# JohnLonginotto/uq

Hardware: AMD Instinct MI355X
Metric: FASTQ encode MB/s (150bp synthetic; bit-exact tables vs reference) (higher is better)
Workload: dtype u8

## Files before the change

include/uqhip.h:

```cpp
#ifndef UQHIP_H
#define UQHIP_H
#include <stddef.h>
#include <stdint.h>

#ifdef __cplusplus
extern "C" {
#endif

#define UQ_ABI_VERSION 1
#define UQ_NONE UINT64_MAX

typedef struct uq_ctx uq_ctx;

const char* uq_last_error(void);
int uq_abi_version(void);
int uq_device_count(int* h_count);
int uq_ctx_create(int device, void* stream, uq_ctx** out);
int uq_ctx_destroy(uq_ctx* ctx);
int uq_ctx_reserve(uq_ctx* ctx, size_t scratch_bytes);
int uq_ctx_sync(uq_ctx* ctx);
int uq_dev_alloc(uq_ctx* ctx, size_t bytes, void** d_out);
int uq_dev_free(uq_ctx* ctx, void* d_ptr);
int uq_h2d(uq_ctx* ctx, void* d_dst, const void* h_src, size_t bytes);
int uq_d2h(uq_ctx* ctx, void* h_dst, const void* d_src, size_t bytes);
// ... 149 lines not shown
int uq_owner_of_rows(uq_ctx* ctx, const int64_t* d_row_index, uint64_t n, const int64_t* h_shard_starts, uint32_t world, uint8_t* d_owner);
int uq_index_affine(uq_ctx* ctx, const void* d_in, int in_itemsize, uint64_t n, int64_t add, void* d_out, int out_itemsize);
int uq_invert_permutation(uq_ctx* ctx, const void* d_perm, int perm_itemsize, uint64_t n, int64_t base, uint32_t* d_inv, uint64_t* h_bad);
int uq_scatter_rows(uq_ctx* ctx, const uint8_t* d_values, uint64_t n, uint32_t cols, const void* d_index, int index_itemsize, int64_t base,
                    uint64_t out_rows, uint8_t* d_out, uint64_t* h_bad);

#define UQ_QF_MAXC 8
#define UQ_QF_MAXT 24
typedef struct uq_qname_fused {
    uint32_t ok, plen, slen, nsep, l1len;
    uint32_t flags;
    uint32_t sample_step, nth;
    uint8_t line1[256];
    uint8_t seps[32];
    uint8_t inset[256];
    uint32_t vmin[UQ_QF_MAXC], vmax[UQ_QF_MAXC];
    uint32_t undetermined[UQ_QF_MAXC];
    uint64_t nreads;
    uint64_t thresholds[UQ_QF_MAXT];
    uint64_t counts[UQ_QF_MAXC][UQ_QF_MAXT];
} uq_qname_fused;
int uq_qname_guess(uq_ctx* ctx, const uint8_t* d_buf, const uint64_t* d_line_start, uint64_t nreads, uq_qname_fused* d_q);
int uq_qname_guess_async(uq_ctx* ctx, const uint8_t* d_buf, const uint64_t* d_line_start, uq_qname_fused* d_q);
int uq_pack_stats_qname(uq_ctx* ctx, const uint8_t* d_buf, const uint64_t* d_line_start, uint64_t first_read, uint64_t nreads,
                        const uq_pack_params* h_guess, uint8_t* d_dna, uint8_t* d_qual, uint64_t* d_bad, uq_stats* d_stats,
                        uq_qname_fused* d_q, uint32_t* d_vals, uint64_t vals_pitch, int* h_fused);
int uq_pack_stats_qname_async(uq_ctx* ctx, const uint8_t* d_buf, const uint64_t* d_line_start, uint64_t capacity_reads,
                              const uq_pack_params* h_guess, uint8_t* d_dna, uint8_t* d_qual, uint64_t* d_bad, uq_stats* d_stats,
                              uq_qname_fused* d_q, uint32_t* d_vals, uint64_t vals_pitch, int* h_fused);
int uq_qname_fused_finish(uq_ctx* ctx, uq_qname_fused* d_q, const uint32_t* d_vals, uint64_t vals_pitch);
int uq_qname_fused_fetch(uq_ctx* ctx, const uq_qname_fused* d_q, uq_qname_fused* h_out);
int uq_qname_fused_first_seen(uq_ctx* ctx, const uint32_t* d_vals, uint64_t vals_pitch, uint64_t nreads, uint64_t read_offset,
                              const uint32_t* h_vmin, const uint32_t* h_range, int ncols, int64_t* d_first);
int uq_encode_u32(uq_ctx* ctx, const uint32_t* d_val, uint64_t n, uint32_t sub, int itemsize, void* d_out);
int uq_encode_u32_columns(uq_ctx* ctx, const uint32_t* d_vals, uint64_t vals_pitch, uint64_t n, int ncols, const uint32_t* h_sub,
                          const int* h_itemsize, void* const* h_d_outs);

typedef struct uq_decisions {
    uint32_t status, nbases, nquals, nall, nnq, ncand;
    uint8_t bases[256], qualities[256], all_bases[256];
    uint8_t nq_base[256]; int32_t nq_code[256];
    int32_t total_quals, bits_per_base, bits_per_quality, variable, dna_max, dna_min, dna_bytes_per_row, quality_bytes_per_row;
    uint64_t base_tot[256], qual_tot[256];
} uq_decisions;
int uq_decide_from_stats(const uq_stats_compact* h_compact, const uint64_t* h_dense, uint32_t len_min, uint32_t len_max, int notricks, int pad,
                         const uint64_t* h_first_seen, uq_decisions* h_out);
// ... 112 lines not shown
```

uq_amd/_lib.py:

```python
import ctypes as C
import os

HERE = os.path.dirname(os.path.abspath(__file__))
LIB_PATH = os.environ.get('UQ_LIB_PATH') or os.path.join(HERE, 'libuqhip.so')
UQ_NONE = (1 << 64) - 1
ABI_VERSION = 1


class UqHipError(RuntimeError):
    pass


class Stats(C.Structure):
    _fields_ = [('counts', C.c_uint64 * 65536), ('bad_plus', C.c_uint64), ('bad_len', C.c_uint64),
                ('len_min', C.c_uint32), ('len_max', C.c_uint32), ('max_record_bytes', C.c_uint32),
                ('reserved', C.c_uint32)]


class PackParams(C.Structure):
    _fields_ = [('dna_code', C.c_int16 * 256), ('qual_code', C.c_int16 * 256), ('n_qual', C.c_int32 * 256),
                ('bits_per_base', C.c_int32), ('bits_per_quality', C.c_int32), ('variable', C.c_int32),
                ('dna_bytes_per_row', C.c_int32), ('quality_bytes_per_row', C.c_int32),
                ('max_record_bytes', C.c_int32), ('dna_max', C.c_int32), ('avg_record_bytes', C.c_int32)]

# ... 124 lines not shown
    'uq_narrow': [_vp, _vp, _u64, _int, _vp],
    'uq_stack_columns': [_vp, _P(_vp), _P(_int), _int, _u64, _int, _vp],
    'uq_unstack_column': [_vp, _vp, _u64, _int, _int, _int, _int, _vp],
    'uq_unpack': [_vp, _vp, _vp, _u64, _P(UnpackParams), _vp, _vp, _vp, _vp],
    'uq_qname_analyse': [_vp, _vp, _u64, _P(_vp), _P(_int)],
    'uq_qname_json': [_vp, _P(C.c_char_p)],
    'uq_qname_column': [_vp, _int, _vp, _u64],
    'uq_qname_free': [_vp],
    'uq_qname_layout': [_vp, _vp, _vp, _u64, _u64, _vp, _u32, _P(QnameLayoutResult)],
    'uq_qname_tokenise': [_vp, _vp, _vp, _u64, _u32, _u32, _vp, _u32, _P(_vp), _P(_vp), _P(QnameColsResult)],
    'uq_prefix_distinct': [_vp, _vp, _int, _vp, _u64, _P(_u64), _int, _P(_u64)],
    'uq_int_prefix_distinct': [_vp, _vp, _u64, C.c_int64, _u64, _u64, _P(_u64), _int, _P(_u64)],
    'uq_encode_int': [_vp, _vp, _u64, C.c_int64, _int, _vp],
    'uq_unique_sorted_rows': [_vp, _vp, _u64, _u32, _vp, _vp, _P(_u64)],
    'uq_unique_rows_of_groups': [_vp, _vp, _u64, _u32, _vp, _vp, _u64, _vp],
    'uq_partition_order': [_vp, _vp, _u64, _u32, _vp, _vp, _P(_u64)],
    'uq_partition_rows': [_vp, _vp, _u32, _u32, _vp, _u64, _u64, _u64, _vp],
    'uq_owner_of_rows': [_vp, _vp, _u64, _P(C.c_int64), _u32, _vp],
    'uq_index_affine': [_vp, _vp, _int, _u64, C.c_int64, _vp, _int],
    'uq_invert_permutation': [_vp, _vp, _int, _u64, C.c_int64, _vp, _P(_u64)],
    'uq_scatter_rows': [_vp, _vp, _u64, _u32, _vp, _int, C.c_int64, _u64, _vp, _P(_u64)],
    'uq_qname_guess': [_vp, _vp, _vp, _u64, _vp],
    'uq_qname_guess_async': [_vp, _vp, _vp, _vp],
    'uq_pack_stats_qname': [_vp, _vp, _vp, _u64, _u64, _P(PackParams), _vp, _vp, _vp, _vp, _vp, _vp, _u64, _P(_int)],
    'uq_pack_stats_qname_async': [_vp, _vp, _vp, _u64, _P(PackParams), _vp, _vp, _vp, _vp, _vp, _vp, _u64, _P(_int)],
    'uq_qname_fused_finish': [_vp, _vp, _vp, _u64],
    'uq_qname_fused_fetch': [_vp, _vp, _P(QnameFused)],
    'uq_qname_fused_first_seen': [_vp, _vp, _u64, _u64, _u64, _P(_u32), _P(_u32), _int, _vp],
    'uq_encode_u32': [_vp, _vp, _u64, _u32, _int, _vp],
    'uq_encode_u32_columns': [_vp, _vp, _u64, _u64, _int, _P(_u32), _P(_int), _P(_vp)],
    'uq_decide_from_stats': [_vp, _vp, _u32, _u32, _int, _int, _vp, _P(Decisions)],
    'uq_make_pack_params': [C.c_char_p, _u32, C.c_char_p, _u32, C.c_char_p, _P(C.c_int32), _u32] + [C.c_int32] * 8 + [_P(PackParams)],
    'uq_same_pack_params': [_P(PackParams), _P(PackParams), _P(_int)],
    'uq_qname_fused_columns': [_P(QnameFused), _u64, _P(QnameColumns)],
    'uq_emit_fastq': [_vp, _P(EmitParams), _P(_vp), _P(_vp), _P(_vp), _vp, _vp, _vp, _u64, _vp, _vp, _u64, _P(_u64)],
    'uq_debug_scribble_lds': [_vp, C.c_uint32],
    'uq_sort_config': [_vp, C.c_int64, _P(_int), _int],
    'uq_sort_counters': [_vp, _P(_u64), _P(_u64)],
    'uq_decode_fastq': [_vp, _P(EmitParams), _P(UnpackParams), _P(_vp), _P(_vp), _P(_vp), _vp, _vp, _u64, _vp, _vp, _vp, _vp, _u64, _P(_u64), _P(_u64)],
    'uq_synth_size': [_vp, _P(SynthSpec), _u64, _u64, _P(_u64)],
    'uq_synth_fastq': [_vp, _P(SynthSpec), _u64, _u64, _vp, _u64],
    'uq_gzip_scan': [_vp, _u64, _vp, _u64, _P(_u64), _P(_u64), _P(_int), _P(_u64)],
    'uq_inflate_members': [_vp, _vp, _u64, _vp, _u64, _vp, _u64, _vp],
    'uq_inflate_member_host': [_vp, _u64, _vp, _u64, _u32, _P(_u32)],
    'uq_gzip_stream_begin': [_vp, _vp, _u64, _u64, _vp, _u64, _P(_vp), _P(_u64), _P(_u32), _P(_u64)],
    'uq_gzip_stream_finish': [_vp, _vp, _u64, _P(_u32), _P(_u64)],
# ... 54 lines not shown
```

uq_amd/csrc/api.hip:

```cpp
#include <stdarg.h>
#include "common.h"

static thread_local char g_err[1024] = "";

void uq_set_error(const char* fmt, ...) {
    va_list ap;
    va_start(ap, fmt);
    vsnprintf(g_err, sizeof(g_err), fmt, ap);
    va_end(ap);
}

extern "C" const char* uq_last_error(void) { return g_err; }
extern "C" int uq_abi_version(void) { return UQ_ABI_VERSION; }

extern "C" int uq_device_count(int* h_count) {
    UQ_REQUIRE(h_count, "uq_device_count: null out pointer");
    UQ_CHECK_HIP(hipGetDeviceCount(h_count));
    return 0;
}

extern "C" int uq_ctx_create(int device, void* stream, uq_ctx** out) {
    UQ_REQUIRE(out, "uq_ctx_create: null out pointer");
    int n = 0;
    UQ_CHECK_HIP(hipGetDeviceCount(&n));
// ... 5 lines not shown
    if (stream) { c->stream = (hipStream_t)stream; c->own_stream = false; }
    else { UQ_CHECK_HIP(hipStreamCreateWithFlags(&c->stream, hipStreamNonBlocking)); c->own_stream = true; }
    UQ_CHECK_HIP(hipEventCreate(&c->ev0));
    UQ_CHECK_HIP(hipEventCreate(&c->ev1));
    UQ_CHECK_HIP(hipHostMalloc((void**)&c->h_pinned, 131072, hipHostMallocDefault));
    UQ_CHECK_HIP(hipHostGetDevicePointer((void**)&c->d_pinned, c->h_pinned, 0));
    UQ_CHECK_HIP(hipMalloc((void**)&c->d_async, 64));
    *out = c;
    return 0;
}

extern "C" int uq_ctx_destroy(uq_ctx* c) {
    if (!c) return 0;
    (void)hipSetDevice(c->device);
    (void)hipStreamSynchronize(c->stream);
    if (c->scratch) (void)hipFree(c->scratch);
    if (c->idx_partials) (void)hipFree(c->idx_partials);
    if (c->idx_bitmap) (void)hipFree(c->idx_bitmap);
    if (c->scan_ws) (void)hipFree(c->scan_ws);
    if (c->h_pinned) (void)hipHostFree(c->h_pinned);
    if (c->d_async) (void)hipFree(c->d_async);
    if (c->qf_first) (void)hipFree(c->qf_first);
    if (c->qf_lay) (void)hipFree(c->qf_lay);
    if (c->d_compact) (void)hipFree(c->d_compact);
    (void)hipEventDestroy(c->ev0);
    (void)hipEventDestroy(c->ev1);
    if (c->own_stream) (void)hipStreamDestroy(c->stream);
    delete c;
    return 0;
}

namespace {
__global__ void read_back_kernel(const uint32_t* __restrict__ src, uint32_t* __restrict__ dst, uint32_t nwords) {
    for (uint32_t i = blockIdx.x * blockDim.x + threadIdx.x; i < nwords; i += gridDim.x * blockDim.x) dst[i] = src[i];
}
}

int uq_read_back(uq_ctx* c, void* h_dst, const void* d_src, size_t bytes) {
    const size_t off = (size_t)((const uint8_t*)h_dst - (const uint8_t*)c->h_pinned);
    UQ_REQUIRE(bytes % 4 == 0 && off % 4 == 0 && off + bytes <= 131072, "uq_read_back: destination outside the pinned staging buffer");
    if (bytes == 0) return 0;
    const uint32_t nwords = (uint32_t)(bytes / 4);
    read_back_kernel<<<nwords > 1024 ? 8 : 1, 256, 0, c->stream>>>((const uint32_t*)d_src, (uint32_t*)((uint8_t*)c->d_pinned + off), nwords);
    UQ_LAUNCH_CHECK();
    return 0;
}
// ... 93 lines not shown
```

uq_amd/csrc/common.h:

```cpp
#pragma once
#include <hip/hip_runtime.h>
#include <stdint.h>
#include <stdio.h>
#include <string.h>
#include "../../include/uqhip.h"

#define UQ_WAVE 64
#define UQ_NUM_CU 256

struct uq_ctx {
    int device;
    hipStream_t stream;
    bool own_stream;
    void* scratch;
    size_t scratch_bytes;
    hipEvent_t ev0, ev1;
    const uint8_t* idx_buf; uint64_t idx_nbytes; uint64_t idx_nlines;
    uint32_t* idx_partials; size_t idx_partials_cap;
    uint16_t* idx_bitmap;
    uint64_t* h_pinned;
    uint64_t* d_pinned;
    void* scan_ws; size_t scan_ws_bytes;
    unsigned long long* d_async;
    const uint8_t* async_buf; uint64_t async_nbytes; bool async_read;
    bool census_begun; uint64_t census_nb;
    uint32_t* qf_first;
    void* qf_lay; bool qf_lay_dirty;
    bool qf_dirty;
    const void* pk_stats; const void* pk_q; const void* stats_sent;
    uq_stats_compact* d_compact;
    const void* qf_sent;
    long long msd_min_rows; int msd_levels; int msd_bits[4];
    unsigned long long n_msd_rounds, n_lsd_rounds;
    const void* kreg_key[8]; int kreg_val[8]; int kreg_n;
    bool qf_attr_set;
};

void uq_set_error(const char* fmt, ...);

#define UQ_CHECK_HIP(expr)                                                              \
    do {                                                                                \
        hipError_t _e = (expr);                                                         \
        if (_e != hipSuccess) {                                                         \
            uq_set_error("%s failed: %s (%s:%d)", #expr, hipGetErrorString(_e), __FILE__, __LINE__); \
            return 1;                                                                   \
        }                                                                               \
    } while (0)

#define UQ_REQUIRE(cond, ...)                                                           \
    do {                                                                                \
// ... 88 lines not shown
```

uq_amd/csrc/qname_fused.hip:

```cpp
#include "common.h"
#include "lines.h"
#include "stats_compact.h"

namespace {
constexpr int QF_THREADS = 256;
constexpr int QF_MAXCH = 64;
constexpr uint32_t QF_SAMPLES = 4096;
constexpr uint32_t QF_ROW = 64, QF_STRIDE = QF_ROW + 4;
constexpr uint32_t QF_FT = 1u << 20;
constexpr uint32_t QF_SMALL = 4096;
constexpr size_t QF_PINNED_AT = 5200;
static_assert(sizeof(uq_qname_fused) % 4 == 0 && QF_PINNED_AT * 8 + sizeof(uq_qname_fused) <= 8000 * 8, "the structure's slot in the pinned staging");
constexpr uint64_t QF_PREFIX = 1ull << 21;

struct DevLine1 {
    uint8_t text[256];
    uint8_t slot[256];
    uint8_t ch[QF_MAXCH];
    uint16_t cnt[QF_MAXCH];
    uint16_t lastpos[QF_MAXCH];
    uint32_t len, nch, bad, pad;
};

__device__ __forceinline__ void stage_line(uint8_t* row, const uint8_t* q, uint32_t ql, const uint8_t* buf_end) {
    for (uint32_t c = 0; c < ql; c += 16) {
        if (q + c + 16 <= buf_end) {
            uint4 v;
            __builtin_memcpy(&v, q + c, 16);
            uint32_t* d = (uint32_t*)(row + c);
            d[0] = v.x; d[1] = v.y; d[2] = v.z; d[3] = v.w;
        } else {
            for (uint32_t b = c; b < ql; ++b) row[b] = q[b];
        }
    }
}

constexpr uint32_t QF_SPW = 8;
__global__ __launch_bounds__(64) void qname_sample_kernel(const uint8_t* __restrict__ buf, const uint64_t* __restrict__ ls, uint64_t n,
                                                                   const unsigned long long* __restrict__ d_async, uq_qname_layout_result* __restrict__ lay,
                                                                   DevLine1* __restrict__ l1_out, uint32_t* __restrict__ step_out, CensusView cv, uint64_t nbytes,
                                                                   const uint32_t* __restrict__ over) {
    __shared__ __align__(16) uint8_t stage[64 * QF_STRIDE];
    __shared__ DevLine1 l1;
    __shared__ unsigned long long s_entry[QF_MAXCH], s_viol[QF_MAXCH];
    __shared__ uint32_t s_lcp, s_lcs, s_flags;
    const uint32_t tid = threadIdx.x;
    const bool lists = cv.list != nullptr;
    uint64_t nlines = 4 * n;
    if (d_async) { nlines = d_async[0]; n = (d_async[1] || (lists && *over)) ? 0 : d_async[0] / 4; }
    uint32_t len = 0;
    if (n) { bool ok; const uint64_t e = lists ? cv_line_start(cv, nlines, 0, 0, 1, ok) : ls[1]; len = e >= 1 && e <= 256 ? (uint32_t)(e - 1) : 0xFFFFFFFFu; }
    for (uint32_t x = tid; x < 256; x += 64) { l1.text[x] = (len != 0xFFFFFFFFu && x < len) ? buf[x] : 0; l1.slot[x] = 0xFF; }
    if (tid < QF_MAXCH) { l1.ch[tid] = 0; l1.cnt[tid] = 0; l1.lastpos[tid] = 0; s_entry[tid] = UQ_NONE; s_viol[tid] = 0; }
    if (tid == 0) { s_lcp = 0xFFFFFFFFu; s_lcs = 0xFFFFFFFFu; s_flags = 0; }
    __syncthreads();
    const bool bad0 = len == 0 || len == 0xFFFFFFFFu || l1.text[0] != '@';
    if (!bad0 && len <= 64) {
        const uint32_t lane0 = lane_id();
        const uint32_t mych = lane0 < len ? (uint32_t)l1.text[lane0] : 0x100u;
        unsigned long long same = 0;
        for (uint32_t j = 0; j < len; ++j) {
            const unsigned long long bm = __ballot(mych == (uint32_t)__builtin_amdgcn_readlane((int)mych, (int)j));
            if (lane0 == j) same = bm;
        }
        const bool first = lane0 < len && (uint32_t)__builtin_ctzll(same | (1ull << 63)) == lane0;
        const unsigned long long fm = __ballot(first);
        if (first) {
            const uint32_t sl = (uint32_t)__popcll(fm & ((1ull << lane0) - 1));
            l1.slot[mych] = (uint8_t)sl; l1.ch[sl] = (uint8_t)mych;
            l1.cnt[sl] = (uint16_t)__popcll(same); l1.lastpos[sl] = (uint16_t)(63 - __builtin_clzll(same));
        }
        if (lane0 == 0) { l1.len = len; l1.nch = (uint32_t)__popcll(fm); l1.bad = 0; l1.pad = 0; }
    } else if (tid == 0) {
        uint32_t nch = 0, bad = bad0 ? 1u : 0u;
        if (!bad)
            for (uint32_t p = 0; p < len; ++p) {
                const uint8_t c = l1.text[p];
                if (l1.slot[c] == 0xFF) {
                    if (nch == QF_MAXCH) { bad = 1; break; }
                    l1.slot[c] = (uint8_t)nch; l1.ch[nch] = c; ++nch;
                }
                l1.cnt[l1.slot[c]] += 1; l1.lastpos[l1.slot[c]] = (uint16_t)p;
            }
        l1.len = bad ? 0 : len; l1.nch = nch; l1.bad = bad; l1.pad = 0;
    }
    __syncthreads();
    const uint32_t step = (uint32_t)(n / QF_SAMPLES > 1 ? n / QF_SAMPLES : 1);
    if (blockIdx.x == 0) {
        for (uint32_t i = tid; i < sizeof(DevLine1) / 4; i += 64) ((uint32_t*)l1_out)[i] = ((const uint32_t*)&l1)[i];
        if (tid == 0) *step_out = step;
    }
    if (l1.bad) return;
    const uint8_t* buf_end = lists ? buf + nbytes : buf + ls[4 * n];
    const uint64_t ks = lists ? (uint64_t)QF_SAMPLES : 0;
    uint32_t my_lcp = 0xFFFFFFFFu, my_lcs = 0xFFFFFFFFu;
    const uint32_t lane = lane_id();
    const uint32_t my_ch = lane < l1.nch ? l1.ch[lane] : 0x100u;
    const uint32_t my_cnt = lane < l1.nch ? l1.cnt[lane] : 0u, my_last = lane < l1.nch ? l1.lastpos[lane] : 0u;
    for (uint64_t k0 = (uint64_t)blockIdx.x * QF_SPW; lists ? k0 < ks : k0 * step < n; k0 += (uint64_t)gridDim.x * QF_SPW) {
        const uint64_t k = k0 + lane;
        uint64_t h = (k + 0x9E3779B97F4A7C15ull) * 0xBF58476D1CE4E5B9ull;
        h ^= h >> 29; h *= 0x94D049BB133111EBull; h ^= h >> 32;
        uint64_t i = lists ? 0 : k * step + h % step;
        uint64_t q0 = 0, q1 = 0;
        if (lists) {
            if (lane < QF_SPW && k < ks) {
                const uint64_t T = (((k << 16) | (h & 0xFFFFu)) * cv.nb) / (ks << 16);
                const uint64_t o = cv.offs[T], c = (T + 1 < cv.nb ? (uint64_t)cv.offs[T + 1] : nlines) - o;
                uint32_t slot = (3u - (uint32_t)o) & 3u;
                if (c > slot) slot += 4u * (uint32_t)((h >> 16) % ((c - slot + 3) / 4));
                const uint64_t rank = o + slot;
                bool ok0, ok1;
                q0 = cv_line_start(cv, nlines, (uint32_t)T, slot + 1, 0, ok0); q1 = cv_line_start(cv, nlines, (uint32_t)T, slot + 1, 1, ok1);
                if (ok0 && ok1) i = (rank + 1) / 4;
            }
        } else if (lane < QF_SPW && i && i < n) { q0 = ls[4 * i]; q1 = ls[4 * i + 1]; }
        if (lane >= QF_SPW || i >= n) i = 0;
        const uint8_t* q = buf;
        uint32_t ql = 0;
        uint8_t* row = stage + tid * QF_STRIDE;
        if (i) {
            q = buf + q0;
            ql = (uint32_t)(q1 - q0 - 1);
            if (ql <= QF_ROW) stage_line(row, q, ql, buf_end);
        }
        for (uint32_t sidx = 0; sidx < QF_SPW; ++sidx) {
            const uint64_t si = __shfl(i, sidx, 64);
            if (si == 0) continue;
            const uint32_t sql = (uint32_t)__shfl(ql, sidx, 64);
            if (sql > 255) { if (lane == 0) atomicOr(&s_flags, 2u); continue; }
            const uint8_t* sq = (const uint8_t*)__shfl((unsigned long long)(uintptr_t)q, sidx, 64);
            const uint8_t* srow = stage + sidx * QF_STRIDE;
            const uint32_t m = sql < l1.len ? sql : l1.len;
            uint32_t lcp = m, last_bad = 0xFFFFFFFFu, have = 0;
            bool lcp_open = true;
            for (uint32_t base = 0; base < sql; base += 64) {
                const uint32_t pos = base + lane;
                const bool valid = pos < sql;
                const uint32_t b = valid ? (sql <= QF_ROW ? srow[pos] : sq[pos]) : 0x100u;
                const unsigned long long pm = __ballot(valid && pos < m && b != l1.text[pos]);
                if (lcp_open && pm) { lcp = base + (uint32_t)__builtin_ctzll(pm); lcp_open = false; }
                const uint32_t t = sql - 1 - pos;
                const unsigned long long sm = __ballot(valid && t < m && b != l1.text[l1.len - 1 - t]);
                if (sm) last_bad = base + 63u - (uint32_t)__builtin_clzll(sm);
                for (uint32_t c = 0; c < l1.nch; ++c) {
                    const unsigned long long cm = __ballot(b == (uint32_t)l1.ch[c]);
                    if (lane == c) have += (uint32_t)__popcll(cm);
                }
            }
            const uint32_t lcs = last_bad == 0xFFFFFFFFu ? m : sql - 1 - last_bad;
            if (lane == 0 && ((lcp == sql && sql < l1.len) || (lcs == sql && sql < l1.len))) atomicOr(&s_flags, 1u);
            if (lcp < my_lcp) my_lcp = lcp;
            if (lcs < my_lcs) my_lcs = lcs;
            if (lane < l1.nch) {
                if (lcp <= my_last && (unsigned long long)si < s_entry[lane]) atomicMin(&s_entry[lane], (unsigned long long)si);
                if (have != my_cnt && (unsigned long long)si > s_viol[lane]) atomicMax(&s_viol[lane], (unsigned long long)si);
            }
        }
    }
    (void)my_ch;
    if (lane_id() == 0) { atomicMin(&s_lcp, my_lcp); atomicMin(&s_lcs, my_lcs); }
    __syncthreads();
    if (tid < l1.nch) {
        if (s_entry[tid] != UQ_NONE) atomicMin((unsigned long long*)&lay->entry[tid], s_entry[tid]);
        if (s_viol[tid]) atomicMax((unsigned long long*)&lay->lastviol[tid], s_viol[tid]);
    }
    if (tid == 0) {
        atomicMin(&lay->min_lcp, s_lcp); atomicMin(&lay->min_lcs, s_lcs);
        if (s_flags) atomicOr(&lay->flags, s_flags);
    }
}

__global__ void layout_init_kernel(uq_qname_layout_result* lay) {
    const uint32_t t = threadIdx.x;
    if (t < QF_MAXCH) { lay->entry[t] = UQ_NONE; lay->lastviol[t] = 0; lay->ch[t] = 0; }
    if (t == 0) { lay->min_lcp = 0xFFFFFFFFu; lay->min_lcs = 0xFFFFFFFFu; lay->flags = 0; lay->nch = 0; }
}

__device__ bool regex_special(uint8_t c) {
    const char* s = ".^$*+?{}[]\\|()-";
    for (int i = 0; s[i]; ++i) if ((uint8_t)s[i] == c) return true;
    return false;
}

__global__ void qname_guess_kernel(const DevLine1* __restrict__ g_l1, uq_qname_layout_result* __restrict__ g_lay, const uint32_t* __restrict__ step,
                                   uq_qname_fused* __restrict__ q) {
    __shared__ DevLine1 s_l1;
    __shared__ uq_qname_layout_result s_lay;
    for (uint32_t i = threadIdx.x; i < sizeof(DevLine1) / 4; i += 64) ((uint32_t*)&s_l1)[i] = ((const uint32_t*)g_l1)[i];
    for (uint32_t i = threadIdx.x; i < sizeof(uq_qname_layout_result) / 4; i += 64) ((uint32_t*)&s_lay)[i] = ((const uint32_t*)g_lay)[i];
    __syncthreads();
    {
        const uint32_t t0 = threadIdx.x;
        if (t0 < QF_MAXCH) { g_lay->entry[t0] = UQ_NONE; g_lay->lastviol[t0] = 0; g_lay->ch[t0] = 0; }
        if (t0 == 0) { g_lay->min_lcp = 0xFFFFFFFFu; g_lay->min_lcs = 0xFFFFFFFFu; g_lay->flags = 0; g_lay->nch = 0; }
    }
    const DevLine1* l1 = &s_l1;
    const uq_qname_layout_result* lay = &s_lay;
    const uint32_t t = threadIdx.x;
    for (uint32_t i = t; i < 256; i += 64) { q->line1[i] = i < l1->len ? l1->text[i] : 0; q->inset[i] = 0; }
    if (t < 32) q->seps[t] = 0;
    if (t < UQ_QF_MAXC) { q->vmin[t] = 0xFFFFFFFFu; q->vmax[t] = 0; q->undetermined[t] = 0; }
    for (uint32_t i = t; i < UQ_QF_MAXC * UQ_QF_MAXT; i += 64) (&q->counts[0][0])[i] = 0;
    if (t < UQ_QF_MAXT) q->thresholds[t] = 0;
    if (t == 0) { q->ok = 0; q->plen = q->slen = q->nsep = q->l1len = 0; q->flags = 0; q->sample_step = *step; q->nth = 0; q->nreads = 0; }
    if (l1->bad || lay->flags) return;
    const uint32_t len = l1->len;
    const uint32_t plen = lay->min_lcp < len ? lay->min_lcp : len, slen = lay->min_lcs < len ? lay->min_lcs : len;
    if (plen == 0 || plen + slen > len) return;
    __shared__ uint8_t s_sep[QF_MAXCH];
    bool mine = false, special = false;
    if (t < l1->nch && lay->entry[t] != UQ_NONE && lay->lastviol[t] < lay->entry[t]) {
        const uint8_t c = l1->ch[t];
        int mid = 0, ord = 0;
        for (uint32_t p = plen; p < len - slen; ++p) { mid += l1->text[p] == c; ord += (p + 1 < len - slen) && l1->text[p] == c; }
        mine = mid != 0;
        special = mine && regex_special(c);
        if (mine && (ord != mid || (c >= '0' && c <= '9'))) special = true;
    }
    s_sep[t] = mine ? 1 : 0;
    const uint32_t nsepch = (uint32_t)__popcll(__ballot(mine));
    if (__ballot(special) || nsepch == 0 || nsepch > 4) return;
    __syncthreads();
    if (t != 0) return;
    uint32_t nsep = 0;
    const uint32_t end = len - slen >= 1 ? len - slen - 1 : 0;
    for (uint32_t p = plen; p < end; ++p) {
        const uint8_t c = l1->text[p];
        if (l1->slot[c] != 0xFF && s_sep[l1->slot[c]]) {
            if (nsep == UQ_QF_MAXC - 1) return;
            q->seps[nsep++] = c;
        }
    }
    if (nsep == 0) return;
    __builtin_amdgcn_s_waitcnt(0);
    for (uint32_t k = 0; k < l1->nch; ++k) if (s_sep[k]) q->inset[l1->ch[k]] = 1;
    q->plen = plen; q->slen = slen; q->nsep = nsep; q->l1len = len;
    q->ok = 1;
}

struct Checkpoints { uint64_t t[UQ_QF_MAXT]; uint32_t nth, nhead; };
__device__ __forceinline__ Checkpoints checkpoints(uint64_t n) {
    Checkpoints c; c.nth = 0; c.nhead = 0;
    if (n == 0) return c;
    for (uint64_t t = 10000; t <= n - 1 && c.nth < UQ_QF_MAXT - 1; t *= 2) c.t[c.nth++] = t;
    if (c.nth == 0 || c.t[c.nth - 1] != n - 1) c.t[c.nth++] = n - 1;
    for (uint32_t k = 0; k < c.nth; ++k) if (c.t[k] < QF_PREFIX) c.nhead = k + 1;
    return c;
}

__global__ __launch_bounds__(QF_THREADS) void qf_first_seen_kernel(uq_qname_fused* __restrict__ q, const uint32_t* __restrict__ vals, uint64_t pitch,
                                                                    uint32_t* __restrict__ first, uint32_t* __restrict__ compact_n) {
    __shared__ uint32_t s_first[QF_SMALL];
    const uint32_t col = blockIdx.y;
    if (compact_n && blockIdx.x == 0 && col == 0 && threadIdx.x == 0) *compact_n = 0;
    if (!q->ok || q->flags || col > q->nsep) return;
    const uint64_t n = q->nreads;
    const uint32_t vmin = q->vmin[col], vmax = q->vmax[col];
    if (n == 0 || vmin > vmax) return;
    const uint64_t range = (uint64_t)vmax - vmin + 1;
    if (range > QF_SMALL) return;
// ... 132 lines not shown
    const uint32_t* over = nullptr;
    if (use_lists) {
        cv.mis = (uint32_t)((uintptr_t)d_buf & 15);
        cv.list = ctx->idx_bitmap; cv.offs = ctx->idx_partials;
        cv.nb = (((ctx->async_nbytes + cv.mis + 15) / 16) * 16 + CV_TILE - 1) / CV_TILE;
        over = (const uint32_t*)(ctx->idx_bitmap + cv.nb * CV_LIST_CAP);
    }
    ScratchPlan sp;
    const size_t o_l1 = sp.add(sizeof(DevLine1)), o_step = sp.add(16);
    void* scr;
    UQ_TRY(uq_scratch(ctx, sp.off, &scr));
    uint8_t* base = (uint8_t*)scr;
    if (!ctx->qf_lay) { UQ_CHECK_HIP(hipMalloc(&ctx->qf_lay, sizeof(uq_qname_layout_result))); ctx->qf_lay_dirty = true; }
    uq_qname_layout_result* d_lay = (uq_qname_layout_result*)ctx->qf_lay;
    if (ctx->qf_lay_dirty) {
        layout_init_kernel<<<1, 256, 0, ctx->stream>>>(d_lay);
        UQ_LAUNCH_CHECK();
    }
    ctx->qf_lay_dirty = true;
    const uint32_t grid = QF_SAMPLES / QF_SPW;
    qname_sample_kernel<<<grid, 64, 0, ctx->stream>>>(d_buf, d_line_start, nreads, d_async, d_lay, (DevLine1*)(base + o_l1), (uint32_t*)(base + o_step), cv,
                                                      use_lists ? ctx->async_nbytes : 0, over);
    UQ_LAUNCH_CHECK();
    qname_guess_kernel<<<1, 64, 0, ctx->stream>>>((const DevLine1*)(base + o_l1), d_lay, (const uint32_t*)(base + o_step), d_q);
    UQ_LAUNCH_CHECK();
    ctx->qf_lay_dirty = false;
    return 0;
}
}

extern "C" int uq_qname_guess(uq_ctx* ctx, const uint8_t* d_buf, const uint64_t* d_line_start, uint64_t nreads, uq_qname_fused* d_q) {
    return guess_impl(ctx, d_buf, d_line_start, nreads, nullptr, d_q);
}

extern "C" int uq_qname_guess_async(uq_ctx* ctx, const uint8_t* d_buf, const uint64_t* d_line_start, uq_qname_fused* d_q) {
    UQ_REQUIRE(ctx && ctx->async_buf == d_buf, "uq_qname_guess_async: not the buffer of the last uq_count_lines_end_async");
    return guess_impl(ctx, d_buf, d_line_start, 0, ctx->d_async, d_q);
}

extern "C" int uq_qname_fused_finish(uq_ctx* ctx, uq_qname_fused* d_q, const uint32_t* d_vals, uint64_t vals_pitch) {
    UQ_REQUIRE(ctx && d_q && d_vals, "uq_qname_fused_finish: null argument");
    const uq_stats* st = ctx->pk_q == (const void*)d_q ? (const uq_stats*)ctx->pk_stats : nullptr;
    ctx->pk_stats = ctx->pk_q = nullptr;
    const size_t bytes = (size_t)UQ_QF_MAXC * QF_SMALL * sizeof(uint32_t);
    if (!ctx->qf_first) { UQ_CHECK_HIP(hipMalloc((void**)&ctx->qf_first, bytes)); ctx->qf_dirty = true; }
    if (!ctx->d_compact) UQ_CHECK_HIP(hipMalloc((void**)&ctx->d_compact, sizeof(uq_stats_compact)));
    if (ctx->qf_dirty) UQ_CHECK_HIP(hipMemsetAsync(ctx->qf_first, 0xFF, bytes, ctx->stream));
    ctx->qf_dirty = true;
    if (!ctx->qf_attr_set) { UQ_CHECK_HIP(hipFuncSetAttribute((const void*)qf_epilogue_kernel, hipFuncAttributeMaxDynamicSharedMemorySize, (int)(QF_FT / 8))); ctx->qf_attr_set = true; }
    qf_first_seen_kernel<<<dim3(UQ_NUM_CU * 4, UQ_QF_MAXC), QF_THREADS, 0, ctx->stream>>>(d_q, d_vals, vals_pitch, ctx->qf_first, st ? &ctx->d_compact->n : nullptr);
    UQ_LAUNCH_CHECK();
    qf_epilogue_kernel<<<EP_WG, QF_THREADS, QF_FT / 8, ctx->stream>>>(d_q, ctx->qf_first, d_vals, vals_pitch, st, ctx->d_compact);
    UQ_LAUNCH_CHECK();
    ctx->qf_dirty = false;
    Gather g;
    memset(&g, 0, sizeof(g));
    g.s[0] = GatherSeg{(const uint32_t*)d_q, (uint32_t*)(ctx->d_pinned + QF_PINNED_AT), (uint32_t)(sizeof(uq_qname_fused) / 4), 0};
    const uint32_t *d_async, *d_over;
    const bool census = uq_async_sources(ctx, &d_async, &d_over);
    if (census) {
// ... 124 lines not shown
```

uq_amd/ops.py:

```python
import ctypes as C

import numpy as np

from ._lib import call, Stats, PackParams, UnpackParams, SynthSpec, GzipStreamInfo, BgzfPart, Fingerprint, UQ_NONE, load

PATTERN_IDS = {'0.1': 0, '0.2': 1, '1.1': 2, '1.2': 3, '2.1': 4, '2.2': 5, '3.1': 6, '3.2': 7}


def _p(t):
    return C.c_void_p(t.data_ptr()) if t is not None else C.c_void_p(0)


def count_lines(ctx, buf):
    n = C.c_uint64()
    call('uq_count_lines', ctx.h, _p(buf), buf.numel(), C.byref(n))
    return n.value


class ChunkedCensus:

    def __init__(self, ctx, buf):
        self.ctx, self.buf = ctx, buf
        call('uq_count_lines_begin', ctx.h, _p(buf), buf.numel())

# ... 286 lines not shown

QF_MAXC = 8


class FusedQname:

    def __init__(self, ctx, capacity_reads):
        from ._lib import QnameFused
        t = ctx.torch
        self.pitch = (int(capacity_reads) + 3) & ~3
        self.q = t.empty(C.sizeof(QnameFused), dtype=t.uint8, device=ctx.device)
        self.vals = t.empty(QF_MAXC * self.pitch, dtype=t.int32, device=ctx.device)

    def column(self, c, n):
        return self.vals[c * self.pitch:c * self.pitch + n]


def qname_guess(ctx, buf, line_start, nreads, fq):
    call('uq_qname_guess', ctx.h, _p(buf), _p(line_start), int(nreads), _p(fq.q))


def qname_guess_async(ctx, buf, line_start, fq):
    call('uq_qname_guess_async', ctx.h, _p(buf), _p(line_start), _p(fq.q))


def qname_fused_finish(ctx, fq):
    call('uq_qname_fused_finish', ctx.h, _p(fq.q), _p(fq.vals), fq.pitch)


def qname_fused_fetch(ctx, fq):
    from ._lib import QnameFused
    out = QnameFused()
    call('uq_qname_fused_fetch', ctx.h, _p(fq.q), C.byref(out))
    return out


def qname_fused_first_seen(ctx, fq, n, read_offset, vmins, ranges):
    t = ctx.torch
    k = len(vmins)
    first = t.empty(QF_MAXC * 4096, dtype=t.int64, device=ctx.device)
    call('uq_qname_fused_first_seen', ctx.h, _p(fq.vals), fq.pitch, int(n), int(read_offset), (C.c_uint32 * k)(*[int(x) for x in vmins]),
         (C.c_uint32 * k)(*[int(x) for x in ranges]), k, _p(first))
    return first


def encode_u32_columns(ctx, fq, n, subs, itemsizes):
# ... 599 lines not shown
```

Before: 1.525 million.

## Guess qname layout from byte-position samples on a side stream

Adds a position-based sampling kernel that picks random byte windows, finds FASTQ record boundaries inside them, and runs the qname layout guess on a separate non-blocking stream without waiting for the line census. If the guess holds on at least half the samples it is used directly; otherwise the code falls back to the census-based path. This is meant to take the guess off the critical path that waits on line counting, for inputs above a size threshold of about 3 GB. It adds a host-side stream synchronize and the risk of a wrong layout guess when windows land badly, and the threshold means small inputs never take the new path.

After: 1.550 million, median of 6. +1.6%, better.

```diff
diff --git a/include/uqhip.h b/include/uqhip.h
--- a/include/uqhip.h
+++ b/include/uqhip.h
@@ -195,6 +195,10 @@
 } uq_qname_fused;
 int uq_qname_guess(uq_ctx* ctx, const uint8_t* d_buf, const uint64_t* d_line_start, uint64_t nreads, uq_qname_fused* d_q);
 int uq_qname_guess_async(uq_ctx* ctx, const uint8_t* d_buf, const uint64_t* d_line_start, uq_qname_fused* d_q);
+int uq_qname_guess_last_form(uq_ctx* ctx, int* h_form);
+int uq_qname_guess_config(uq_ctx* ctx, int64_t beside_min_bytes);
+int uq_qname_guess_stats(uq_ctx* ctx, uint32_t* h_out4);
+int uq_qname_guess_list_async(uq_ctx* ctx, const uint8_t* d_buf, uq_qname_fused* d_q);
 int uq_pack_stats_qname(uq_ctx* ctx, const uint8_t* d_buf, const uint64_t* d_line_start, uint64_t first_read, uint64_t nreads,
                         const uq_pack_params* h_guess, uint8_t* d_dna, uint8_t* d_qual, uint64_t* d_bad, uq_stats* d_stats,
                         uq_qname_fused* d_q, uint32_t* d_vals, uint64_t vals_pitch, int* h_fused);
diff --git a/uq_amd/_lib.py b/uq_amd/_lib.py
--- a/uq_amd/_lib.py
+++ b/uq_amd/_lib.py
@@ -170,6 +170,10 @@
     'uq_scatter_rows': [_vp, _vp, _u64, _u32, _vp, _int, C.c_int64, _u64, _vp, _P(_u64)],
     'uq_qname_guess': [_vp, _vp, _vp, _u64, _vp],
     'uq_qname_guess_async': [_vp, _vp, _vp, _vp],
+    'uq_qname_guess_last_form': [_vp, _vp],
+    'uq_qname_guess_config': [_vp, C.c_int64],
+    'uq_qname_guess_stats': [_vp, _vp],
+    'uq_qname_guess_list_async': [_vp, _vp, _vp],
     'uq_pack_stats_qname': [_vp, _vp, _vp, _u64, _u64, _P(PackParams), _vp, _vp, _vp, _vp, _vp, _vp, _u64, _P(_int)],
     'uq_pack_stats_qname_async': [_vp, _vp, _vp, _u64, _P(PackParams), _vp, _vp, _vp, _vp, _vp, _vp, _u64, _P(_int)],
     'uq_qname_fused_finish': [_vp, _vp, _vp, _u64],
diff --git a/uq_amd/csrc/api.hip b/uq_amd/csrc/api.hip
--- a/uq_amd/csrc/api.hip
+++ b/uq_amd/csrc/api.hip
@@ -51,6 +51,8 @@
     if (c->d_async) (void)hipFree(c->d_async);
     if (c->qf_first) (void)hipFree(c->qf_first);
     if (c->qf_lay) (void)hipFree(c->qf_lay);
+    if (c->qf_stream) { (void)hipStreamSynchronize(c->qf_stream); (void)hipStreamDestroy(c->qf_stream); }
+    if (c->qf_side) (void)hipFree(c->qf_side);
     if (c->d_compact) (void)hipFree(c->d_compact);
     (void)hipEventDestroy(c->ev0);
     (void)hipEventDestroy(c->ev1);
diff --git a/uq_amd/csrc/common.h b/uq_amd/csrc/common.h
--- a/uq_amd/csrc/common.h
+++ b/uq_amd/csrc/common.h
@@ -26,6 +26,10 @@
     bool census_begun; uint64_t census_nb;
     uint32_t* qf_first;
     void* qf_lay; bool qf_lay_dirty;
+    hipStream_t qf_stream; void* qf_side; bool qf_side_dirty;
+    long long qf_beside_min;
+    uint32_t qf_stat[4];
+    int qf_form;
     bool qf_dirty;
     const void* pk_stats; const void* pk_q; const void* stats_sent;
     uq_stats_compact* d_compact;
diff --git a/uq_amd/csrc/qname_fused.hip b/uq_amd/csrc/qname_fused.hip
--- a/uq_amd/csrc/qname_fused.hip
+++ b/uq_amd/csrc/qname_fused.hip
@@ -35,25 +35,7 @@
     }
 }
 
-constexpr uint32_t QF_SPW = 8;
-__global__ __launch_bounds__(64) void qname_sample_kernel(const uint8_t* __restrict__ buf, const uint64_t* __restrict__ ls, uint64_t n,
-                                                                   const unsigned long long* __restrict__ d_async, uq_qname_layout_result* __restrict__ lay,
-                                                                   DevLine1* __restrict__ l1_out, uint32_t* __restrict__ step_out, CensusView cv, uint64_t nbytes,
-                                                                   const uint32_t* __restrict__ over) {
-    __shared__ __align__(16) uint8_t stage[64 * QF_STRIDE];
-    __shared__ DevLine1 l1;
-    __shared__ unsigned long long s_entry[QF_MAXCH], s_viol[QF_MAXCH];
-    __shared__ uint32_t s_lcp, s_lcs, s_flags;
-    const uint32_t tid = threadIdx.x;
-    const bool lists = cv.list != nullptr;
-    uint64_t nlines = 4 * n;
-    if (d_async) { nlines = d_async[0]; n = (d_async[1] || (lists && *over)) ? 0 : d_async[0] / 4; }
-    uint32_t len = 0;
-    if (n) { bool ok; const uint64_t e = lists ? cv_line_start(cv, nlines, 0, 0, 1, ok) : ls[1]; len = e >= 1 && e <= 256 ? (uint32_t)(e - 1) : 0xFFFFFFFFu; }
-    for (uint32_t x = tid; x < 256; x += 64) { l1.text[x] = (len != 0xFFFFFFFFu && x < len) ? buf[x] : 0; l1.slot[x] = 0xFF; }
-    if (tid < QF_MAXCH) { l1.ch[tid] = 0; l1.cnt[tid] = 0; l1.lastpos[tid] = 0; s_entry[tid] = UQ_NONE; s_viol[tid] = 0; }
-    if (tid == 0) { s_lcp = 0xFFFFFFFFu; s_lcs = 0xFFFFFFFFu; s_flags = 0; }
-    __syncthreads();
+__device__ __forceinline__ void sample_line1_table(DevLine1& l1, const uint32_t len, const uint32_t tid) {
     const bool bad0 = len == 0 || len == 0xFFFFFFFFu || l1.text[0] != '@';
     if (!bad0 && len <= 64) {
         const uint32_t lane0 = lane_id();
@@ -84,6 +66,73 @@
             }
         l1.len = bad ? 0 : len; l1.nch = nch; l1.bad = bad; l1.pad = 0;
     }
+}
+
+struct SampleAcc { unsigned long long entry[QF_MAXCH], viol[QF_MAXCH]; uint32_t lcp, lcs, flags; };
+__device__ __forceinline__ void sample_reduce_line(const DevLine1& l1, SampleAcc& acc, const unsigned long long si, const uint32_t sql, const uint8_t* srow,
+                                                   const uint8_t* sq, const uint32_t lane, const uint32_t my_cnt, const uint32_t my_last, uint32_t& my_lcp,
+                                                   uint32_t& my_lcs) {
+    if (sql > 255) { if (lane == 0) atomicOr(&acc.flags, 2u); return; }
+    const uint32_t m = sql < l1.len ? sql : l1.len;
+    uint32_t lcp = m, last_bad = 0xFFFFFFFFu, have = 0;
+    bool lcp_open = true;
+    for (uint32_t base = 0; base < sql; base += 64) {
+        const uint32_t pos = base + lane;
+        const bool valid = pos < sql;
+        const uint32_t b = valid ? (srow ? srow[pos] : sq[pos]) : 0x100u;
+        const unsigned long long pm = __ballot(valid && pos < m && b != l1.text[pos]);
+        if (lcp_open && pm) { lcp = base + (uint32_t)__builtin_ctzll(pm); lcp_open = false; }
+        const uint32_t t = sql - 1 - pos;
+        const unsigned long long sm = __ballot(valid && t < m && b != l1.text[l1.len - 1 - t]);
+        if (sm) last_bad = base + 63u - (uint32_t)__builtin_clzll(sm);
+        for (uint32_t c = 0; c < l1.nch; ++c) {
+            const unsigned long long cm = __ballot(b == (uint32_t)l1.ch[c]);
+            if (lane == c) have += (uint32_t)__popcll(cm);
+        }
+    }
+    const uint32_t lcs = last_bad == 0xFFFFFFFFu ? m : sql - 1 - last_bad;
+    if (lane == 0 && ((lcp == sql && sql < l1.len) || (lcs == sql && sql < l1.len))) atomicOr(&acc.flags, 1u);
+    if (lcp < my_lcp) my_lcp = lcp;
+    if (lcs < my_lcs) my_lcs = lcs;
+    if (lane < l1.nch) {
+        if (lcp <= my_last && si < acc.entry[lane]) atomicMin(&acc.entry[lane], si);
+        if (have != my_cnt && si > acc.viol[lane]) atomicMax(&acc.viol[lane], si);
+    }
+}
+
+__device__ __forceinline__ void sample_flush(const DevLine1& l1, SampleAcc& acc, const uint32_t my_lcp, const uint32_t my_lcs, uq_qname_layout_result* __restrict__ lay,
+                                             const uint32_t tid) {
+    if (lane_id() == 0) { atomicMin(&acc.lcp, my_lcp); atomicMin(&acc.lcs, my_lcs); }
+    __syncthreads();
+    if (tid < l1.nch) {
+        if (acc.entry[tid] != UQ_NONE) atomicMin((unsigned long long*)&lay->entry[tid], acc.entry[tid]);
+        if (acc.viol[tid]) atomicMax((unsigned long long*)&lay->lastviol[tid], acc.viol[tid]);
+    }
+    if (tid == 0) {
+        atomicMin(&lay->min_lcp, acc.lcp); atomicMin(&lay->min_lcs, acc.lcs);
+        if (acc.flags) atomicOr(&lay->flags, acc.flags);
+    }
+}
+
+constexpr uint32_t QF_SPW = 8;
+__global__ __launch_bounds__(64) void qname_sample_kernel(const uint8_t* __restrict__ buf, const uint64_t* __restrict__ ls, uint64_t n,
+                                                                   const unsigned long long* __restrict__ d_async, uq_qname_layout_result* __restrict__ lay,
+                                                                   DevLine1* __restrict__ l1_out, uint32_t* __restrict__ step_out, CensusView cv, uint64_t nbytes,
+                                                                   const uint32_t* __restrict__ over) {
+    __shared__ __align__(16) uint8_t stage[64 * QF_STRIDE];
+    __shared__ DevLine1 l1;
+    __shared__ SampleAcc acc;
+    const uint32_t tid = threadIdx.x;
+    const bool lists = cv.list != nullptr;
+    uint64_t nlines = 4 * n;
+    if (d_async) { nlines = d_async[0]; n = (d_async[1] || (lists && *over)) ? 0 : d_async[0] / 4; }
+    uint32_t len = 0;
+    if (n) { bool ok; const uint64_t e = lists ? cv_line_start(cv, nlines, 0, 0, 1, ok) : ls[1]; len = e >= 1 && e <= 256 ? (uint32_t)(e - 1) : 0xFFFFFFFFu; }
+    for (uint32_t x = tid; x < 256; x += 64) { l1.text[x] = (len != 0xFFFFFFFFu && x < len) ? buf[x] : 0; l1.slot[x] = 0xFF; }
+    if (tid < QF_MAXCH) { l1.ch[tid] = 0; l1.cnt[tid] = 0; l1.lastpos[tid] = 0; acc.entry[tid] = UQ_NONE; acc.viol[tid] = 0; }
+    if (tid == 0) { acc.lcp = 0xFFFFFFFFu; acc.lcs = 0xFFFFFFFFu; acc.flags = 0; }
+    __syncthreads();
+    sample_line1_table(l1, len, tid);
     __syncthreads();
     const uint32_t step = (uint32_t)(n / QF_SAMPLES > 1 ? n / QF_SAMPLES : 1);
     if (blockIdx.x == 0) {
@@ -95,7 +144,6 @@
     const uint64_t ks = lists ? (uint64_t)QF_SAMPLES : 0;
     uint32_t my_lcp = 0xFFFFFFFFu, my_lcs = 0xFFFFFFFFu;
     const uint32_t lane = lane_id();
-    const uint32_t my_ch = lane < l1.nch ? l1.ch[lane] : 0x100u;
     const uint32_t my_cnt = lane < l1.nch ? l1.cnt[lane] : 0u, my_last = lane < l1.nch ? l1.lastpos[lane] : 0u;
     for (uint64_t k0 = (uint64_t)blockIdx.x * QF_SPW; lists ? k0 < ks : k0 * step < n; k0 += (uint64_t)gridDim.x * QF_SPW) {
         const uint64_t k = k0 + lane;
@@ -128,47 +176,87 @@
             const uint64_t si = __shfl(i, sidx, 64);
             if (si == 0) continue;
             const uint32_t sql = (uint32_t)__shfl(ql, sidx, 64);
-            if (sql > 255) { if (lane == 0) atomicOr(&s_flags, 2u); continue; }
             const uint8_t* sq = (const uint8_t*)__shfl((unsigned long long)(uintptr_t)q, sidx, 64);
-            const uint8_t* srow = stage + sidx * QF_STRIDE;
-            const uint32_t m = sql < l1.len ? sql : l1.len;
-            uint32_t lcp = m, last_bad = 0xFFFFFFFFu, have = 0;
-            bool lcp_open = true;
-            for (uint32_t base = 0; base < sql; base += 64) {
-                const uint32_t pos = base + lane;
-                const bool valid = pos < sql;
-                const uint32_t b = valid ? (sql <= QF_ROW ? srow[pos] : sq[pos]) : 0x100u;
-                const unsigned long long pm = __ballot(valid && pos < m && b != l1.text[pos]);
-                if (lcp_open && pm) { lcp = base + (uint32_t)__builtin_ctzll(pm); lcp_open = false; }
-                const uint32_t t = sql - 1 - pos;
-                const unsigned long long sm = __ballot(valid && t < m && b != l1.text[l1.len - 1 - t]);
-                if (sm) last_bad = base + 63u - (uint32_t)__builtin_clzll(sm);
-                for (uint32_t c = 0; c < l1.nch; ++c) {
-                    const unsigned long long cm = __ballot(b == (uint32_t)l1.ch[c]);
-                    if (lane == c) have += (uint32_t)__popcll(cm);
-                }
+            sample_reduce_line(l1, acc, si, sql, sql <= QF_ROW ? stage + sidx * QF_STRIDE : nullptr, sq, lane, my_cnt, my_last, my_lcp, my_lcs);
+        }
+    }
+    sample_flush(l1, acc, my_lcp, my_lcs, lay, tid);
+}
+
+constexpr uint32_t QF_WIN = 2048;
+__global__ __launch_bounds__(64) void qname_sample_pos_kernel(const uint8_t* __restrict__ buf, const uint64_t nbytes, uq_qname_layout_result* __restrict__ lay,
+                                                              DevLine1* __restrict__ l1_out, uint32_t* __restrict__ step_out) {
+    __shared__ __align__(16) uint8_t s_win[QF_SPW * QF_WIN];
+    __shared__ DevLine1 l1;
+    __shared__ SampleAcc acc;
+    const uint32_t tid = threadIdx.x, lane = tid;
+    const uint64_t k0 = (uint64_t)blockIdx.x * QF_SPW;
+    uint32_t head[4] = {0, 0, 0, 0};
+    uint4 wv[2 * QF_SPW];
+    const uint64_t k = k0 + lane;
+    uint64_t h = (k + 0x9E3779B97F4A7C15ull) * 0xBF58476D1CE4E5B9ull;
+    h ^= h >> 29; h *= 0x94D049BB133111EBull; h ^= h >> 32;
+    const uint64_t sw = nbytes / QF_SAMPLES;
+    const uint64_t my_ws = sw ? k * sw + h % sw : k * nbytes / QF_SAMPLES;
+#pragma unroll
+    for (uint32_t j = 0; j < 4; ++j) if (j * 64 + tid < nbytes) head[j] = buf[j * 64 + tid];
+#pragma unroll
+    for (uint32_t s = 0; s < QF_SPW; ++s) {
+        const uint64_t ws = __shfl(my_ws, s, 64);
+        const bool live = k0 + s < QF_SAMPLES;
+#pragma unroll
+        for (uint32_t j = 0; j < 2; ++j) {
+            const uint64_t at = ws + j * (QF_WIN / 2) + tid * 16;
+            uint8_t tmp[16] = {0};
+            if (live && at + 16 <= nbytes) __builtin_memcpy(tmp, buf + at, 16);
+            else for (uint32_t b = 0; b < 16; ++b) if (live && at + b < nbytes) tmp[b] = buf[at + b];
+            __builtin_memcpy(&wv[2 * s + j], tmp, 16);
+        }
+    }
+    uint32_t len = nbytes ? 0xFFFFFFFFu : 0;
+#pragma unroll
+    for (uint32_t j = 0; j < 4; ++j) {
+        const unsigned long long nl = __ballot(j * 64 + tid < nbytes && head[j] == '\n');
+        if (nl && len == 0xFFFFFFFFu) len = j * 64 + (uint32_t)__builtin_ctzll(nl);
+    }
+#pragma unroll
+    for (uint32_t j = 0; j < 4; ++j) { const uint32_t x = j * 64 + tid; l1.text[x] = (len != 0xFFFFFFFFu && x < len) ? (uint8_t)head[j] : 0; l1.slot[x] = 0xFF; }
+    if (tid < QF_MAXCH) { l1.ch[tid] = 0; l1.cnt[tid] = 0; l1.lastpos[tid] = 0; acc.entry[tid] = UQ_NONE; acc.viol[tid] = 0; }
+    if (tid == 0) { acc.lcp = 0xFFFFFFFFu; acc.lcs = 0xFFFFFFFFu; acc.flags = 0; }
+    __syncthreads();
+    sample_line1_table(l1, len, tid);
+    __syncthreads();
+    if (blockIdx.x == 0) {
+        for (uint32_t i = tid; i < sizeof(DevLine1) / 4; i += 64) ((uint32_t*)l1_out)[i] = ((const uint32_t*)&l1)[i];
+        if (tid == 0) step_out[0] = 0;
+    }
+    if (l1.bad) return;
+    uint32_t my_lcp = 0xFFFFFFFFu, my_lcs = 0xFFFFFFFFu;
+    const uint32_t my_cnt = lane < l1.nch ? l1.cnt[lane] : 0u, my_last = lane < l1.nch ? l1.lastpos[lane] : 0u;
+#pragma unroll
+    for (uint32_t x = 0; x < 2 * QF_SPW; ++x) *(uint4*)(s_win + (x >> 1) * QF_WIN + (x & 1) * (QF_WIN / 2) + lane * 16) = wv[x];
+    __syncthreads();
+    uint32_t nfound = 0;
+    for (uint32_t s = 0; s < QF_SPW && k0 + s < QF_SAMPLES; ++s) {
+        const uint64_t ws = __shfl(my_ws, s, 64);
+        const uint8_t* w = s_win + s * QF_WIN;
+        const uint32_t wl = nbytes - ws < QF_WIN ? (uint32_t)(nbytes - ws) : QF_WIN;
+        uint32_t n0 = 0xFFFFFFFFu, n1 = 0xFFFFFFFFu, n2 = 0xFFFFFFFFu, n3 = 0xFFFFFFFFu;
+        bool found = false;
+        for (uint32_t base = 0; base < wl && !found; base += 64) {
+            unsigned long long nl = __ballot(base + lane < wl && w[base + lane] == '\n');
+            while (nl && !found) {
+                n0 = n1; n1 = n2; n2 = n3; n3 = base + (uint32_t)__builtin_ctzll(nl);
+                nl &= nl - 1;
+                found = n0 != 0xFFFFFFFFu && w[n0 + 1] == '@' && w[n2 + 1] == '+';
             }
-            const uint32_t lcs = last_bad == 0xFFFFFFFFu ? m : sql - 1 - last_bad;
-            if (lane == 0 && ((lcp == sql && sql < l1.len) || (lcs == sql && sql < l1.len))) atomicOr(&s_flags, 1u);
-            if (lcp < my_lcp) my_lcp = lcp;
-            if (lcs < my_lcs) my_lcs = lcs;
-            if (lane < l1.nch) {
-                if (lcp <= my_last && (unsigned long long)si < s_entry[lane]) atomicMin(&s_entry[lane], (unsigned long long)si);
-                if (have != my_cnt && (unsigned long long)si > s_viol[lane]) atomicMax(&s_viol[lane], (unsigned long long)si);
-            }
-        }
-    }
-    (void)my_ch;
-    if (lane_id() == 0) { atomicMin(&s_lcp, my_lcp); atomicMin(&s_lcs, my_lcs); }
-    __syncthreads();
-    if (tid < l1.nch) {
-        if (s_entry[tid] != UQ_NONE) atomicMin((unsigned long long*)&lay->entry[tid], s_entry[tid]);
-        if (s_viol[tid]) atomicMax((unsigned long long*)&lay->lastviol[tid], s_viol[tid]);
-    }
-    if (tid == 0) {
-        atomicMin(&lay->min_lcp, s_lcp); atomicMin(&lay->min_lcs, s_lcs);
-        if (s_flags) atomicOr(&lay->flags, s_flags);
-    }
+        }
+        if (!found) continue;
+        ++nfound;
+        sample_reduce_line(l1, acc, ws + n0 + 2, n1 - n0 - 1, w + n0 + 1, nullptr, lane, my_cnt, my_last, my_lcp, my_lcs);
+    }
+    if (lane == 0 && nfound) atomicAdd(step_out + 1, nfound);
+    sample_flush(l1, acc, my_lcp, my_lcs, lay, tid);
 }
 
 __global__ void layout_init_kernel(uq_qname_layout_result* lay) {
@@ -183,8 +271,8 @@
     return false;
 }
 
-__global__ void qname_guess_kernel(const DevLine1* __restrict__ g_l1, uq_qname_layout_result* __restrict__ g_lay, const uint32_t* __restrict__ step,
-                                   uq_qname_fused* __restrict__ q) {
+__global__ void qname_guess_kernel(const DevLine1* __restrict__ g_l1, uq_qname_layout_result* __restrict__ g_lay, uint32_t* __restrict__ step,
+                                   uq_qname_fused* __restrict__ q, uint32_t* __restrict__ note) {
     __shared__ DevLine1 s_l1;
     __shared__ uq_qname_layout_result s_lay;
     for (uint32_t i = threadIdx.x; i < sizeof(DevLine1) / 4; i += 64) ((uint32_t*)&s_l1)[i] = ((const uint32_t*)g_l1)[i];
@@ -204,6 +292,7 @@
     for (uint32_t i = t; i < UQ_QF_MAXC * UQ_QF_MAXT; i += 64) (&q->counts[0][0])[i] = 0;
     if (t < UQ_QF_MAXT) q->thresholds[t] = 0;
     if (t == 0) { q->ok = 0; q->plen = q->slen = q->nsep = q->l1len = 0; q->flags = 0; q->sample_step = *step; q->nth = 0; q->nreads = 0; }
+    if (t == 0 && note) { note[0] = 0; note[1] = step[1]; step[1] = 0; }
     if (l1->bad || lay->flags) return;
     const uint32_t len = l1->len;
     const uint32_t plen = lay->min_lcp < len ? lay->min_lcp : len, slen = lay->min_lcs < len ? lay->min_lcs : len;
@@ -237,6 +326,7 @@
     for (uint32_t k = 0; k < l1->nch; ++k) if (s_sep[k]) q->inset[l1->ch[k]] = 1;
     q->plen = plen; q->slen = slen; q->nsep = nsep; q->l1len = len;
     q->ok = 1;
+    if (note) note[0] = 1;
 }
 
 struct Checkpoints { uint64_t t[UQ_QF_MAXT]; uint32_t nth, nhead; };
@@ -415,11 +505,43 @@
     qname_sample_kernel<<<grid, 64, 0, ctx->stream>>>(d_buf, d_line_start, nreads, d_async, d_lay, (DevLine1*)(base + o_l1), (uint32_t*)(base + o_step), cv,
                                                       use_lists ? ctx->async_nbytes : 0, over);
     UQ_LAUNCH_CHECK();
-    qname_guess_kernel<<<1, 64, 0, ctx->stream>>>((const DevLine1*)(base + o_l1), d_lay, (const uint32_t*)(base + o_step), d_q);
+    qname_guess_kernel<<<1, 64, 0, ctx->stream>>>((const DevLine1*)(base + o_l1), d_lay, (uint32_t*)(base + o_step), d_q, nullptr);
     UQ_LAUNCH_CHECK();
     ctx->qf_lay_dirty = false;
     return 0;
 }
+
+#ifndef QF_GUESS_IN_STREAM
+#ifndef QF_BESIDE_MIN
+#define QF_BESIDE_MIN 3000000000ll
+#endif
+constexpr long long QF_BESIDE_MIN_BYTES = QF_BESIDE_MIN;
+struct QfSide { uq_qname_layout_result lay; DevLine1 l1; uint32_t step[4]; };
+constexpr size_t QF_NOTE_AT = 5600;
+int guess_beside(uq_ctx* ctx, const uint8_t* d_buf, uq_qname_fused* d_q, bool* stands) {
+    *stands = false;
+    if (!ctx->qf_stream) { UQ_CHECK_HIP(hipSetDevice(ctx->device)); UQ_CHECK_HIP(hipStreamCreateWithFlags(&ctx->qf_stream, hipStreamNonBlocking)); }
+    if (!ctx->qf_side) { UQ_CHECK_HIP(hipMalloc(&ctx->qf_side, sizeof(QfSide))); ctx->qf_side_dirty = true; }
+    QfSide* sd = (QfSide*)ctx->qf_side;
+    if (ctx->qf_side_dirty) {
+        layout_init_kernel<<<1, 256, 0, ctx->qf_stream>>>(&sd->lay);
+        UQ_LAUNCH_CHECK();
+        UQ_CHECK_HIP(hipMemsetAsync(sd->step, 0, sizeof(sd->step), ctx->qf_stream));
+    }
+    ctx->qf_side_dirty = true;
+    volatile uint32_t* note = (volatile uint32_t*)(ctx->h_pinned + QF_NOTE_AT);
+    note[0] = 0; note[1] = 0;
+    qname_sample_pos_kernel<<<QF_SAMPLES / QF_SPW, 64, 0, ctx->qf_stream>>>(d_buf, ctx->async_nbytes, &sd->lay, &sd->l1, sd->step);
+    UQ_LAUNCH_CHECK();
+    qname_guess_kernel<<<1, 64, 0, ctx->qf_stream>>>(&sd->l1, &sd->lay, sd->step, d_q, (uint32_t*)(ctx->d_pinned + QF_NOTE_AT));
+    UQ_LAUNCH_CHECK();
+    UQ_CHECK_HIP(hipStreamSynchronize(ctx->qf_stream));
+    ctx->qf_side_dirty = false;
+    *stands = note[0] == 1 && 2 * note[1] >= QF_SAMPLES;
+    ctx->qf_stat[0] += 1; ctx->qf_stat[2] = note[0]; ctx->qf_stat[3] = note[1];
+    return 0;
+}
+#endif
 }
 
 extern "C" int uq_qname_guess(uq_ctx* ctx, const uint8_t* d_buf, const uint64_t* d_line_start, uint64_t nreads, uq_qname_fused* d_q) {
@@ -428,7 +550,40 @@
 
 extern "C" int uq_qname_guess_async(uq_ctx* ctx, const uint8_t* d_buf, const uint64_t* d_line_start, uq_qname_fused* d_q) {
     UQ_REQUIRE(ctx && ctx->async_buf == d_buf, "uq_qname_guess_async: not the buffer of the last uq_count_lines_end_async");
+    ctx->qf_form = 0;
+#ifndef QF_GUESS_IN_STREAM
+    const long long beside_min = ctx->qf_beside_min ? ctx->qf_beside_min : QF_BESIDE_MIN_BYTES;
+    if (!d_line_start && d_buf && d_q && ctx->async_nbytes > 0 && beside_min > 0 && ctx->async_nbytes >= (uint64_t)beside_min) {
+        bool stands;
+        UQ_TRY(guess_beside(ctx, d_buf, d_q, &stands));
+        if (stands) { ctx->qf_form = 1; return 0; }
+    }
+#endif
     return guess_impl(ctx, d_buf, d_line_start, 0, ctx->d_async, d_q);
+}
+
+extern "C" int uq_qname_guess_config(uq_ctx* ctx, int64_t beside_min_bytes) {
+    UQ_REQUIRE(ctx, "uq_qname_guess_config: null context");
+    ctx->qf_beside_min = beside_min_bytes;
+    return 0;
+}
+
+extern "C" int uq_qname_guess_stats(uq_ctx* ctx, uint32_t* h_out4) {
+    UQ_REQUIRE(ctx && h_out4, "uq_qname_guess_stats: null argument");
+    memcpy(h_out4, ctx->qf_stat, sizeof(ctx->qf_stat));
+    return 0;
+}
+
+extern "C" int uq_qname_guess_last_form(uq_ctx* ctx, int* h_form) {
+    UQ_REQUIRE(ctx && h_form, "uq_qname_guess_last_form: null argument");
+    *h_form = ctx->qf_form;
+    return 0;
+}
+
+extern "C" int uq_qname_guess_list_async(uq_ctx* ctx, const uint8_t* d_buf, uq_qname_fused* d_q) {
+    UQ_REQUIRE(ctx && ctx->async_buf == d_buf, "uq_qname_guess_list_async: not the buffer of the last uq_count_lines_end_async");
+    ctx->qf_form = 0;
+    return guess_impl(ctx, d_buf, nullptr, 0, ctx->d_async, d_q);
 }
 
 extern "C" int uq_qname_fused_finish(uq_ctx* ctx, uq_qname_fused* d_q, const uint32_t* d_vals, uint64_t vals_pitch) {
diff --git a/uq_amd/ops.py b/uq_amd/ops.py
--- a/uq_amd/ops.py
+++ b/uq_amd/ops.py
@@ -332,6 +332,26 @@
 
 def qname_guess_async(ctx, buf, line_start, fq):
     call('uq_qname_guess_async', ctx.h, _p(buf), _p(line_start), _p(fq.q))
+
+
+def qname_guess_last_form(ctx):
+    form = C.c_int(-1)
+    call('uq_qname_guess_last_form', ctx.h, C.byref(form))
+    return form.value
+
+
+def qname_guess_config(ctx, beside_min_bytes=0):
+    call('uq_qname_guess_config', ctx.h, int(beside_min_bytes))
+
+
+def qname_guess_stats(ctx):
+    out = (C.c_uint32 * 4)()
+    call('uq_qname_guess_stats', ctx.h, out)
+    return tuple(int(x) for x in out)
+
+
+def qname_guess_list_async(ctx, buf, fq):
+    call('uq_qname_guess_list_async', ctx.h, _p(buf), _p(fq.q))
 
 
 def qname_fused_finish(ctx, fq):
```
